# CristianSimion5/vk-raytracing-engine

Hardware: AMD Instinct MI355X
Metric: Mrays/s (higher is better)
Workload: dtype f32

## Files before the change

include/vkrt.h:

```cpp
#ifndef VKRT_H
#define VKRT_H

#include <stdint.h>
#include "vkrt_host_device.h"

#ifdef __cplusplus
extern "C" {
#endif

#define VKRT_ABI_VERSION 4

enum vkrt_status {
  VKRT_OK = 0,
  VKRT_ERR_INVALID_ARGUMENT = 1,
  VKRT_ERR_NO_DEVICE = 2,
  VKRT_ERR_HIP = 3,
  VKRT_ERR_OUT_OF_MEMORY = 4,
  VKRT_ERR_NOT_BUILT = 5,
  VKRT_ERR_UNSUPPORTED = 6
};

typedef struct vkrt_scene vkrt_scene;

typedef struct vkrt_prim_mesh {
// ... 88 lines not shown
  float    build_ms;
  uint64_t node_bytes;
  uint64_t triangle_bytes;
  uint32_t reference_count;
  uint32_t reserved;
} vkrt_accel_info;

int         vkrt_abi_version(void);
const char* vkrt_last_error(void);
int         vkrt_device_count(void);

int  vkrt_scene_create(const vkrt_scene_desc* desc, int device, vkrt_scene** out);
void vkrt_scene_destroy(vkrt_scene* scene);

enum vkrt_option {
  VKRT_OPT_MODE            = 1,
  VKRT_OPT_BVH_LAYOUT      = 2,
  VKRT_OPT_WF_SUBFRAMES    = 3,
  VKRT_OPT_WF_TRAV_BLOCK   = 4,
  VKRT_OPT_WF_SHARE        = 5,
  VKRT_OPT_TRI_THRESHOLD   = 6,
  VKRT_OPT_WF_SHARE_PERIOD = 7,
  VKRT_OPT_WF_SHARE_FLAGS  = 8,
  VKRT_OPT_GBUFFER_MIPS    = 9,
  VKRT_OPT_WATERTIGHT      = 10,
  VKRT_OPT_SKIP_DEAD_SHADOW_RAYS = 11,
  VKRT_OPT_ANYHIT_DISSOLVE = 12,
  VKRT_OPT_WF_FRAMES_IN_FLIGHT = 13,
  VKRT_OPT_SPLIT_BUDGET    = 14,
  VKRT_OPT_LAST            = 14,
  VKRT_OPT_WF_SAMPLE_SYNC  = 15,
  VKRT_OPT_WF_CAMERA_ROUNDS = 16,
  VKRT_OPT_WF_TRI_LEND = 17,
  VKRT_INFO_ANYHIT_ORDER   = 100,
  VKRT_INFO_SPLIT_BUDGET   = 101
};
int vkrt_scene_set_option(vkrt_scene* scene, int option, int value);
int vkrt_scene_get_option(const vkrt_scene* scene, int option, int* value);

int vkrt_accel_build(vkrt_scene* scene, uint32_t build_flags, void* hip_stream);
int vkrt_accel_get_info(const vkrt_scene* scene, vkrt_accel_info* out);

int vkrt_scene_update_nodes(vkrt_scene* scene, uint32_t first, uint32_t count, const vkrt_node* nodes, void* hip_stream);
int vkrt_accel_refit(vkrt_scene* scene, void* hip_stream);

enum vkrt_memory { VKRT_MEMORY_HOST = 0, VKRT_MEMORY_DEVICE = 1 };
typedef struct vkrt_vertex_update {
  uint32_t struct_size;
  uint32_t first, count;
  uint32_t memory;
  const float* positions;
  const float* normals;
  const float* tangents;
  const float* texcoords0;
} vkrt_vertex_update;
int vkrt_scene_update_vertices(vkrt_scene* scene, const vkrt_vertex_update* update, void* hip_stream);

typedef struct vkrt_ray {
  float origin[3];    float tmin;
  float direction[3]; float tmax;
} vkrt_ray;
typedef struct vkrt_hit {
  float   t, u, v;
  int32_t instance;
  int32_t primitive;
  int32_t prim_mesh;
// ... 154 lines not shown
```

vk-raytracing-engine_amd/abi.py:

```python
import ctypes as C

c_f = C.c_float
c_i = C.c_int32
c_u = C.c_uint32
c_u64 = C.c_uint64


class Mat4(C.Structure):
    _fields_ = [("m", c_f * 16)]


class GlobalUniforms(C.Structure):
    _fields_ = [("viewProj", Mat4), ("viewInverse", Mat4), ("projInverse", Mat4)]


class PushConstantRay(C.Structure):
    _fields_ = [
        ("clearColor", c_f * 4),
        ("frame", c_i),
        ("lightsCount", c_i),
        ("samples", c_i),
        ("depth", c_i),
        ("useShadows", c_i),
        ("useAO", c_i),
# ... 177 lines not shown
assert C.sizeof(VertexUpdate) == 48
assert C.sizeof(Ray) == 32
assert C.sizeof(Hit) == 32
assert C.sizeof(Surface) == 128
assert C.sizeof(InstanceVisibility) == 4
assert C.sizeof(QueryOpts) == 16
assert C.sizeof(MaterialAlpha) == 8

assert C.sizeof(GlobalUniforms) == 192
assert C.sizeof(PushConstantRay) == 44
assert C.sizeof(PrimMeshInfo) == 12
assert C.sizeof(GltfPBRMaterial) == 52
assert C.sizeof(GltfLight) == 32
assert C.sizeof(PrimMesh) == 20
assert C.sizeof(Node) == 68

VKRT_OK, VKRT_ERR_INVALID_ARGUMENT, VKRT_ERR_NO_DEVICE, VKRT_ERR_HIP, VKRT_ERR_OUT_OF_MEMORY, VKRT_ERR_NOT_BUILT, VKRT_ERR_UNSUPPORTED = range(7)
VKRT_BUILD_LBVH_GPU = 0x1
VKRT_BUILD_SAH_HOST = 0x2
VKRT_BUILD_PLOC_GPU = 0x4
VKRT_TRACE_SEED_INDEX_ROW_MAJOR = 0x1
VKRT_TRACE_COUNT_TRAVERSAL = 0x2
VKRT_TRACE_TIME_KERNELS = 0x4
VKRT_TRACE_SAME_SEED_EVERY_FRAME = 0x8
VKRT_ABI_VERSION = 4
VKRT_OPT_MODE, VKRT_OPT_BVH_LAYOUT, VKRT_OPT_WF_SUBFRAMES, VKRT_OPT_WF_TRAV_BLOCK = 1, 2, 3, 4
VKRT_OPT_WF_SHARE, VKRT_OPT_TRI_THRESHOLD, VKRT_OPT_WF_SHARE_PERIOD, VKRT_OPT_WF_SHARE_FLAGS = 5, 6, 7, 8
VKRT_OPT_GBUFFER_MIPS = 9
VKRT_OPT_WATERTIGHT, VKRT_OPT_SKIP_DEAD_SHADOW_RAYS, VKRT_OPT_ANYHIT_DISSOLVE = 10, 11, 12
VKRT_OPT_WF_FRAMES_IN_FLIGHT, VKRT_OPT_SPLIT_BUDGET = 13, 14
VKRT_OPT_WF_SAMPLE_SYNC = 15
VKRT_OPT_WF_CAMERA_ROUNDS = 16
VKRT_OPT_WF_TRI_LEND = 17
VKRT_INFO_ANYHIT_ORDER = 100
VKRT_INFO_SPLIT_BUDGET = 101
VKRT_INSTANCE_FACING_CULL_DISABLE, VKRT_INSTANCE_FLIP_FACING = 0x1, 0x2
VKRT_RAY_OPAQUE, VKRT_RAY_CULL_BACK_FACING, VKRT_RAY_CULL_FRONT_FACING = 0x1, 0x10, 0x20
VKRT_MEMORY_HOST, VKRT_MEMORY_DEVICE = 0, 1
VKRT_SURFACE_GEOMETRY, VKRT_SURFACE_MATERIAL = 0x1, 0x2
VKRT_ALPHA_OPAQUE, VKRT_ALPHA_MASK = 0, 1
VKRT_MULTIHIT_MAX = 16

VKRT_SYMBOLS = [
    "vkrt_abi_version",
    "vkrt_last_error",
    "vkrt_device_count",
    "vkrt_scene_create",
    "vkrt_scene_destroy",
    "vkrt_scene_set_option",
    "vkrt_scene_get_option",
    "vkrt_reserve",
    "vkrt_reserve_frames",
    "vkrt_accel_build",
    "vkrt_accel_get_info",
    "vkrt_scene_update_nodes",
    "vkrt_accel_refit",
    "vkrt_scene_update_vertices",
    "vkrt_intersect",
    "vkrt_occluded",
    "vkrt_scene_set_instance_visibility",
    "vkrt_scene_get_instance_visibility",
    "vkrt_intersect_ex",
    "vkrt_occluded_ex",
    "vkrt_intersect_multi",
    "vkrt_closest_point",
    "vkrt_hit_surface",
    "vkrt_scene_set_material_alpha",
    "vkrt_scene_get_material_alpha",
# ... 127 lines not shown
```

vk-raytracing-engine_amd/csrc/device_scene.h:

```cpp
#pragma once
#include <hip/hip_runtime.h>
#include <stddef.h>
#include <stdint.h>
#include "../../include/vkrt_host_device.h"
#include "device_math.h"

struct DevInstance
{
  float o2w[12];
  float w2o[9];
  int32_t primMesh;
  uint32_t vis;
  int32_t pad;
};
static_assert(sizeof(DevInstance) == 96, "DevInstance");
#define VKRT_VIS_CULL_DISABLE 0x100u
#define VKRT_VIS_FLIP 0x200u
#define VKRT_VIS_MIRRORED 0x10000u

#define VKRT_VERTEX_QUADS 3
#define VKRT_VERTEX_BYTES 48u
struct DevTexRef
{
  uint32_t offset;
// ... 88 lines not shown
#endif
#ifndef VKRT_W8_POSTPONE_ROOM
#define VKRT_W8_POSTPONE_ROOM 0
#endif

#define VKRT_COUNTER_SLOTS 64
struct DevCounters
{
  unsigned long long v[VKRT_COUNTER_SLOTS][VKRT_COUNTER_STRIDE];
};

#define VKRT_TRACE_PUBLIC_FLAGS 0xFu
#define VKRT_FLAG_SKIP_DEAD_SHADOW 0x100u
#define VKRT_FLAG_STORE_STAGED 0x200u
#define VKRT_FLAG_SAMPLE_SYNC 0x400u
#define VKRT_FLAG_CAMERA_ROUNDS 0x800u

struct TraceParams
{
  DevScene sc;
  PushConstantRay pc;
  float viewInverse[16];
  float projInverse[16];
  uint32_t seed;
  uint32_t flags;
  uint32_t fullW, fullH;
  uint32_t stripRows, shardCount, shardIndex;
  uint32_t localRows;
  uint32_t tilesX, tileCount;
  uint32_t tileFirst;
  float* image;
  unsigned int* workCounter;
  DevCounters* counters;
};

struct WfBuffers
{
  unsigned* ctrl;
  float4* planes;
  float4* stage;
  uint32_t capacity;
  uint32_t groups;
  float4* sampleState;
};
```

vk-raytracing-engine_amd/csrc/vkrt_api.cpp:

```cpp
#include <hip/hip_runtime.h>

#include <algorithm>
#include <chrono>
#include <cmath>
#include <cstdarg>
#include <cstdio>
#include <cstdlib>
#include <cstring>
#include <initializer_list>
#include <string>
#include <vector>

#include "../../include/vkrt.h"
#include "bvh_host.h"
#include "dev_buffer.h"
#include "device_scene.h"
#include "kernels.h"
#include "wide_node.h"

#define VKRT_TRI_THRESHOLD_DEFAULT 32
#define VKRT_WF_SHARE_DEFAULT 16
#define VKRT_WF_SHARE_FLAGS_DEFAULT 25
#define VKRT_WF_FRAMES_IN_FLIGHT_DEFAULT 3
#define VKRT_SPLIT_BUDGET_DEFAULT -1
#define VKRT_WF_SAMPLE_SYNC_DEFAULT 1
#define VKRT_WF_CAMERA_ROUNDS_DEFAULT 1
#define VKRT_WF_TRI_LEND_DEFAULT 1
#include "lbvh.h"
#include "refit.h"
#include "vertex_update.h"

namespace {

thread_local std::string g_lastError;

int fail(int code, const char* fmt, ...)
{
  char buf[512];
  va_list ap;
  va_start(ap, fmt);
  vsnprintf(buf, sizeof buf, fmt, ap);
  va_end(ap);
  g_lastError = buf;
  return code;
}

#define HIP_TRY(expr)                                                      \
  do                                                                       \
  {                                                                        \
    std::string m_;                                                        \
    if(const int rc_ = vkrt::hip_status((expr), #expr, m_); rc_ != VKRT_OK) \
      return fail(rc_, "%s", m_.c_str());                                  \
  } while(0)

}

struct vkrt_scene
{
  int device = 0;
  int cuCount = 256;
  std::vector<float> positions;
  std::vector<uint32_t> indices;
  std::vector<vkrt_prim_mesh> primMeshes;
  std::vector<vkrt_node> nodes;
  uint32_t lightCount = 0, materialCount = 0;
  std::vector<float> materialAlpha;
  std::vector<void*> allocs;
  DevScene dev{};
  vkrt::TreeBuffers accel;
  bool built = false;
  vkrt_accel_info info{};
  unsigned int* workCounter = nullptr;
  DevCounters* counters = nullptr;
  hipEvent_t evStart = nullptr, evStop = nullptr;
  bool timed = false;
  void* wfMem = nullptr;
  WfBuffers wf{};
  WfAsync wfAsync{};
  std::vector<hipEvent_t> wfEvents;
  WfTiming wfTiming{};
  bool wfTimed = false;
  int splitResolved = 0;
  int wfTimingRounds = 0;
  std::vector<hipEvent_t> wfPool;
  int opt[VKRT_OPT_WF_TRI_LEND + 1] = {0, 1, 1, 3, 64, VKRT_WF_SHARE_DEFAULT, VKRT_TRI_THRESHOLD_DEFAULT, 0, VKRT_WF_SHARE_FLAGS_DEFAULT, 1, 0, 0, 0,
                                            VKRT_WF_FRAMES_IN_FLIGHT_DEFAULT, VKRT_SPLIT_BUDGET_DEFAULT, VKRT_WF_SAMPLE_SYNC_DEFAULT, VKRT_WF_CAMERA_ROUNDS_DEFAULT,
                                      VKRT_WF_TRI_LEND_DEFAULT};
  bool hasLargeTriangles = false;
  bool wavefront = true;
  bool stale = false;
  bool refitted = false;
  vkrt::RefitScratch refit;
  bool positionsOnDevice = false;
  vkrt::DevBuf vertexStage;
  size_t vertexStageBytes = 0;
  std::vector<vkrt_instance_visibility> vis;
  uint64_t masksPresent[4] = {0, 0, 0, 0};
  vkrt::DevBuf nodeMasks;
  std::vector<vkrt_material_alpha> alpha;
  uint32_t alphaMasks = 0;
  const uint4* surfacePrimMeshes = nullptr;
};

namespace {

template <typename T>
int upload(vkrt_scene* s, const T* src, size_t count, const T** dst)
{
  void* p = nullptr;
  const size_t bytes = std::max<size_t>(count * sizeof(T), 16);
  HIP_TRY(hipMalloc(&p, bytes));
  s->allocs.push_back(p);
  if(count)
    HIP_TRY(hipMemcpy(p, src, count * sizeof(T), hipMemcpyHostToDevice));
  *dst = (const T*)p;
  return VKRT_OK;
}

int checkTransform(const vkrt_node& n, uint32_t i)
{
  for(int k = 0; k < 16; k++)
    if(!std::isfinite(n.worldMatrix[k]))
      return fail(VKRT_ERR_INVALID_ARGUMENT, "node %u: worldMatrix[%d] is not finite", i, k);
  return VKRT_OK;
}

int validate(const vkrt_scene_desc* d)
{
  if(!d)
    return fail(VKRT_ERR_INVALID_ARGUMENT, "desc is NULL");
  if(d->struct_size != sizeof(vkrt_scene_desc))
// ... 58 lines not shown
      const int x0 = cl((int)flx, (int)sw), x1 = cl((int)flx + 1, (int)sw), y0 = cl((int)fly, (int)sh), y1 = cl((int)fly + 1, (int)sh);
      const uint32_t p[4] = {src[(size_t)y0 * sw + x0], src[(size_t)y0 * sw + x1], src[(size_t)y1 * sw + x0], src[(size_t)y1 * sw + x1]};
      uint32_t out = 0;
      for(int c = 0; c < 4; c++)
      {
        const uint32_t base = (srgb && c < 3) ? 0u : 256u;
        const float t00 = lut512[base + ((p[0] >> (8 * c)) & 255u)], t10 = lut512[base + ((p[1] >> (8 * c)) & 255u)];
        const float t01 = lut512[base + ((p[2] >> (8 * c)) & 255u)], t11 = lut512[base + ((p[3] >> (8 * c)) & 255u)];
        float v = (t00 * (1.0f - ax) + t10 * ax) * (1.0f - ay) + (t01 * (1.0f - ax) + t11 * ax) * ay;
        if(srgb && c < 3) v = srgbEncode(v);
        v = v < 0.0f ? 0.0f : (v > 1.0f ? 1.0f : v);
        out |= (uint32_t)(v * 255.0f + 0.5f) << (8 * c);
      }
      dst[(size_t)y * dw + x] = out;
    }
}

bool useWavefront(const vkrt_scene* s) { return s->opt[VKRT_OPT_MODE] == 1; }

int clampOption(int option, int v)
{
  switch(option)
  {
    case VKRT_OPT_MODE: case VKRT_OPT_BVH_LAYOUT: return v ? 1 : 0;
    case VKRT_OPT_WF_SUBFRAMES: case VKRT_OPT_WF_FRAMES_IN_FLIGHT: return std::max(1, std::min(VKRT_WF_MAX_LANES, v));
    case VKRT_OPT_SPLIT_BUDGET: return std::max(-1, std::min(100, v));
    case VKRT_OPT_WF_TRAV_BLOCK: return v == 256 ? 256 : v == 128 ? 128 : 64;
    case VKRT_OPT_WF_SHARE: return std::max(0, std::min(64, v));
    case VKRT_OPT_TRI_THRESHOLD: return std::max(0, std::min(65, v));
    case VKRT_OPT_WF_SHARE_PERIOD: return std::max(0, std::min(255, v));
    case VKRT_OPT_WF_SHARE_FLAGS: return v & 31;
    case VKRT_OPT_GBUFFER_MIPS: case VKRT_OPT_WATERTIGHT: case VKRT_OPT_SKIP_DEAD_SHADOW_RAYS: case VKRT_OPT_ANYHIT_DISSOLVE: case VKRT_OPT_WF_SAMPLE_SYNC:
    case VKRT_OPT_WF_CAMERA_ROUNDS: case VKRT_OPT_WF_TRI_LEND: return v ? 1 : 0;
  }
  return v;
}

void optionsFromEnvironment(vkrt_scene* s)
{
  const char* e;
  if((e = getenv("VKRT_MODE")) && !strcmp(e, "mega")) s->opt[VKRT_OPT_MODE] = 0;
  if((e = getenv("VKRT_BVH")) && !strcmp(e, "bvh2")) s->opt[VKRT_OPT_BVH_LAYOUT] = 0;
  const struct { const char* name; int option; } ints[] = {{"VKRT_WF_SUBFRAMES", VKRT_OPT_WF_SUBFRAMES}, {"VKRT_WF_TRAV_BLOCK", VKRT_OPT_WF_TRAV_BLOCK},
                                                          {"VKRT_WF_SHARE", VKRT_OPT_WF_SHARE}, {"VKRT_TRI_THRESHOLD", VKRT_OPT_TRI_THRESHOLD},
                                                          {"VKRT_WF_SHARE_PERIOD", VKRT_OPT_WF_SHARE_PERIOD}, {"VKRT_WF_SHARE_FLAGS", VKRT_OPT_WF_SHARE_FLAGS},
                                                          {"VKRT_GBUFFER_MIPS", VKRT_OPT_GBUFFER_MIPS}, {"VKRT_WATERTIGHT", VKRT_OPT_WATERTIGHT},
                                                          {"VKRT_SKIP_DEAD_SHADOW_RAYS", VKRT_OPT_SKIP_DEAD_SHADOW_RAYS},
                                                          {"VKRT_ANYHIT_DISSOLVE", VKRT_OPT_ANYHIT_DISSOLVE}, {"VKRT_WF_FRAMES_IN_FLIGHT", VKRT_OPT_WF_FRAMES_IN_FLIGHT},
                                                          {"VKRT_SPLIT_BUDGET", VKRT_OPT_SPLIT_BUDGET}, {"VKRT_WF_SAMPLE_SYNC", VKRT_OPT_WF_SAMPLE_SYNC},
                                                          {"VKRT_WF_CAMERA_ROUNDS", VKRT_OPT_WF_CAMERA_ROUNDS},
                                                          {"VKRT_WF_TRI_LEND", VKRT_OPT_WF_TRI_LEND}};
  for(const auto& k : ints)
    if((e = getenv(k.name)))
      s->opt[k.option] = clampOption(k.option, atoi(e));
}

void freeAccel(vkrt_scene* s)
{
  s->accel = vkrt::TreeBuffers{};
  s->nodeMasks = vkrt::DevBuf{};
  s->built = false;
  s->refit = vkrt::RefitScratch{};
  s->refitted = false;
  s->stale = false;
}

constexpr vkrt_material_alpha kDefaultAlpha = {VKRT_ALPHA_OPAQUE, 0.5f};
constexpr vkrt_instance_visibility kDefaultVisibility = {0xFF, VKRT_INSTANCE_FACING_CULL_DISABLE, 0};

void makeInstance(const vkrt_node& node, const vkrt_instance_visibility& vis, DevInstance& in)
{
  memset(&in, 0, sizeof in);
  for(int r = 0; r < 3; r++)
    for(int c = 0; c < 4; c++)
      in.o2w[r * 4 + c] = node.worldMatrix[c * 4 + r];
  vkrt::invert3x3_rows(in.o2w, in.w2o);
  in.primMesh = node.primMesh;
  const float* m = in.o2w;
  const double det = (double)m[0] * ((double)m[5] * m[10] - (double)m[6] * m[9]) - (double)m[1] * ((double)m[4] * m[10] - (double)m[6] * m[8]) +
                     (double)m[2] * ((double)m[4] * m[9] - (double)m[5] * m[8]);
  in.vis = (uint32_t)vis.mask | ((uint32_t)vis.flags << 8) | (det < 0.0 ? VKRT_VIS_MIRRORED : 0u);
}

void noteMasks(vkrt_scene* s)
{
  memset(s->masksPresent, 0, sizeof s->masksPresent);
  for(const vkrt_instance_visibility& v : s->vis)
// ... 475 lines not shown
  *out = s;
  return VKRT_OK;
}

void vkrt_scene_destroy(vkrt_scene* s)
{
  if(!s)
    return;
  (void)hipSetDevice(s->device);
  freeAccel(s);
  for(void* p : s->allocs)
    (void)hipFree(p);
  if(s->wfMem) (void)hipFree(s->wfMem);
  if(s->wfAsync.count)
  {
    (void)hipEventDestroy(s->wfAsync.fork);
    for(int j = 0; j < s->wfAsync.count; j++)
    {
      (void)hipStreamDestroy(s->wfAsync.streams[j]);
      (void)hipEventDestroy(s->wfAsync.join[j]);
    }
  }
  for(hipEvent_t e : s->wfEvents) (void)hipEventDestroy(e);
  for(hipEvent_t e : s->wfPool) (void)hipEventDestroy(e);
  if(s->evStart) (void)hipEventDestroy(s->evStart);
  if(s->evStop) (void)hipEventDestroy(s->evStop);
  delete s;
}

int vkrt_scene_set_option(vkrt_scene* s, int option, int value)
{
  if(!s)
    return fail(VKRT_ERR_INVALID_ARGUMENT, "scene is NULL");
  if(option < VKRT_OPT_MODE || option > VKRT_OPT_WF_TRI_LEND)
    return fail(VKRT_ERR_INVALID_ARGUMENT, "unknown option %d", option);
  if(clampOption(option, value) != value)
    return fail(VKRT_ERR_INVALID_ARGUMENT, "option %d: value %d out of range", option, value);
  s->opt[option] = value;
  if(option == VKRT_OPT_WF_TRI_LEND && s->built && s->dev.layout == 1u)
    s->dev.shareFlags = (s->dev.shareFlags & ~VKRT_SHARE_TRI_LEND) | (value ? VKRT_SHARE_TRI_LEND : 0u);
  return VKRT_OK;
}

int vkrt_scene_get_option(const vkrt_scene* s, int option, int* value)
{
  if(!s || !value)
    return fail(VKRT_ERR_INVALID_ARGUMENT, "NULL argument");
  if(option == VKRT_INFO_ANYHIT_ORDER)
  {
    *value = s->built ? (int)(s->dev.shareFlags & 6u) : 0;
    return VKRT_OK;
  }
  if(option == VKRT_INFO_SPLIT_BUDGET)
  {
    *value = s->built ? s->splitResolved : 0;
    return VKRT_OK;
  }
  if(option < VKRT_OPT_MODE || option > VKRT_OPT_WF_TRI_LEND)
    return fail(VKRT_ERR_INVALID_ARGUMENT, "unknown option %d", option);
  *value = s->opt[option];
  return VKRT_OK;
}

int vkrt_reserve(vkrt_scene* s, const vkrt_shard* shard, void* hip_stream)
{
  if(!s)
    return fail(VKRT_ERR_INVALID_ARGUMENT, "NULL argument");
  return vkrt_reserve_frames(s, shard, (uint32_t)std::max(1, s->opt[VKRT_OPT_WF_FRAMES_IN_FLIGHT]), hip_stream);
}

int vkrt_reserve_frames(vkrt_scene* s, const vkrt_shard* shard, uint32_t frames_per_call, void* hip_stream)
{
  if(!s || !shard)
    return fail(VKRT_ERR_INVALID_ARGUMENT, "NULL argument");
  if(frames_per_call == 0)
    return fail(VKRT_ERR_INVALID_ARGUMENT, "frames_per_call is 0");
  int rc = checkShard(shard);
  if(rc == VKRT_OK)
    rc = setDevice(s);
  if(rc != VKRT_OK)
    return rc;
  const uint64_t tiles = (uint64_t)((shard->full_width + 7) / 8) * ((vkrt_shard_rows(shard) + 7) / 8);
  if(tiles * 64 >= 0xFFFFFFFFull)
    return fail(VKRT_ERR_UNSUPPORTED, "launch too large");
  const bool wavefront = s->built ? s->wavefront : useWavefront(s);
  if(tiles == 0 || !wavefront)
    return VKRT_OK;
  int rc2 = ensureWorkingSet(s, (uint32_t)tiles * 64u, framesInFlight(s, (int)std::min<uint32_t>(frames_per_call, VKRT_FRAMES_PER_BATCH)), (hipStream_t)hip_stream);
  if(rc2 == VKRT_OK)
    rc2 = ensureEventPool(s, (int)std::min<uint32_t>(frames_per_call, VKRT_FRAMES_PER_BATCH));
  return rc2;
// ... 203 lines not shown
      std::vector<float> records((size_t)r.triCount * 12);
      hipError_t e = hipSuccess;
      if(r.tree.nodeCount) e = hipMemcpy(b2.nodes.data(), r.tree.buf.nodes.get(), b2.nodes.size() * 4, hipMemcpyDeviceToHost);
      if(e == hipSuccess) e = hipMemcpy(records.data(), r.tree.buf.tris.get(), records.size() * 4, hipMemcpyDeviceToHost);
      r.tree.buf = vkrt::TreeBuffers{};
      if(e != hipSuccess)
        return fail(VKRT_ERR_HIP, "LBVH download: %s", hipGetErrorString(e));
      b2.rootRef = r.tree.rootRef;
      b2.maxDepth = r.tree.maxDepth;
      b2.triOrder.resize(r.triCount);
      std::vector<vkrt::FlatTri> tris(r.triCount);
      for(uint32_t k = 0; k < r.triCount; k++)
      {
        b2.triOrder[k] = k;
        tris[k] = vkrt::unpack_triangle(&records[(size_t)k * 12], watertight);
      }
      vkrt::BuiltWide8 w8;
      vkrt::collapse_wide8(b2, tris, w8, watertight);
      if((rc = uploadHostTree(s, tris, nullptr, &w8, dissolvePtr, stream, tree)) != VKRT_OK)
        return rc;
    }
    else
      tree = std::move(r.tree);
  }
  installTree(s, tree);
  sceneBounds(s);
  if((rc = traversalSettings(s)) != VKRT_OK)
    return rc;
  if(s->dev.layout == 1u)
  {
    HIP_TRY(s->nodeMasks.alloc(std::max<size_t>(s->info.node_bytes / VKRT_WNODE_BYTES * 8, 16)));
    if((rc = computeNodeMasks(s, stream)) != VKRT_OK)
      return rc;
  }
  s->info.build_ms = std::chrono::duration<float, std::milli>(std::chrono::steady_clock::now() - t0).count();
  s->built = true;
  return VKRT_OK;
}

}

int vkrt_accel_build(vkrt_scene* s, uint32_t flags, void* hip_stream)
{
  if(!s)
    return fail(VKRT_ERR_INVALID_ARGUMENT, "scene is NULL");
  hipStream_t stream = (hipStream_t)hip_stream;
  if(s->positionsOnDevice)
  {
    int rc = setDevice(s);
    if(rc != VKRT_OK)
      return rc;
    HIP_TRY(hipDeviceSynchronize());
    if(!s->positions.empty())
      HIP_TRY(hipMemcpy(s->positions.data(), s->dev.positions, s->positions.size() * sizeof(float), hipMemcpyDeviceToHost));
    s->positionsOnDevice = false;
  }
  const bool deviceBuild = flags == 0 || (flags & (VKRT_BUILD_LBVH_GPU | VKRT_BUILD_PLOC_GPU)) != 0;
  if(s->opt[VKRT_OPT_SPLIT_BUDGET] >= 0 || !deviceBuild)
  {
    s->splitResolved = std::max(0, s->opt[VKRT_OPT_SPLIT_BUDGET]);
    return accelBuildOnce(s, flags, s->splitResolved, stream);
  }
  const auto t0 = std::chrono::steady_clock::now();
  float sahSplit = 0.0f;
  int rc = accelBuildOnce(s, flags, 30, stream);
  if(rc == VKRT_OK)
// ... 330 lines not shown
  int rc = checkBuilt(s, "vkrt_pathtrace");
  if(rc == VKRT_OK)
    rc = checkShard(shard);
  if(rc != VKRT_OK)
    return rc;
  if(pc->lightsCount < 0 || (uint32_t)pc->lightsCount > s->lightCount)
    return fail(VKRT_ERR_INVALID_ARGUMENT, "PushConstantRay.lightsCount %d outside [0,%u]", pc->lightsCount, s->lightCount);
  if(pc->samples < 0 || pc->depth < 0 || pc->depth > 99)
    return fail(VKRT_ERR_INVALID_ARGUMENT, "samples/depth out of range");
  if((rc = setDevice(s)) != VKRT_OK)
    return rc;
  hipStream_t stream = (hipStream_t)hip_stream;
  TraceParams P;
  if((rc = launchParams(s, pc, cam, opts, shard, P)) != VKRT_OK)
    return rc;
  if(P.localRows == 0)
    return VKRT_OK;
  if(s->opt[VKRT_OPT_SKIP_DEAD_SHADOW_RAYS])
    P.flags |= VKRT_FLAG_SKIP_DEAD_SHADOW;
  P.image = image;
  P.workCounter = s->workCounter;

  const bool count = (P.flags & VKRT_TRACE_COUNT_TRAVERSAL) != 0;
  if(s->wavefront)
  {
    if(P.fullW > 65535u || P.localRows > 65535u || pc->samples > 65535)
      return fail(VKRT_ERR_UNSUPPORTED, "wavefront mode packs pixel coordinates / sample index in 16 bits");
    const uint32_t seedStep = (P.flags & VKRT_TRACE_SAME_SEED_EVERY_FRAME) ? 0u : 1u;
    if(s->opt[VKRT_OPT_WF_SAMPLE_SYNC])
      P.flags |= VKRT_FLAG_SAMPLE_SYNC;
    if(s->opt[VKRT_OPT_WF_CAMERA_ROUNDS] && (P.flags & VKRT_FLAG_SAMPLE_SYNC) && s->dev.layout == 1u && travBlock(s) == 64 && s->dev.shareMinIdle != 0u &&
       s->dev.triThreshold != 0u)
      P.flags |= VKRT_FLAG_CAMERA_ROUNDS;
    if((rc = ensureWorkingSet(s, P.tileCount * 64u, framesInFlight(s, (int)n_frames), stream)) != VKRT_OK)
      return rc;
    if((rc = ensureEventPool(s, (int)std::min<uint32_t>(n_frames, VKRT_FRAMES_PER_BATCH))) != VKRT_OK)
      return rc;
    WfTiming* timing = nullptr;
    if(P.flags & VKRT_TRACE_TIME_KERNELS)
    {
      const size_t wantEv = (size_t)2 * (2 * (size_t)pc->samples * pc->depth) * std::min<uint32_t>(n_frames, 8u);
      while(s->wfEvents.size() < wantEv && s->wfEvents.size() < 8192)
      {
        hipEvent_t e;
        HIP_TRY(hipEventCreate(&e));
        s->wfEvents.push_back(e);
      }
      s->wfTiming.events = s->wfEvents.data();
      s->wfTiming.capacity = (int)s->wfEvents.size();
      timing = &s->wfTiming;
    }
    s->wfTimed = timing != nullptr;
    s->wfTimingRounds = (pc->samples > 0 && pc->depth > 0) ? pc->samples * (pc->depth + 1) : 0;
    HIP_TRY(hipEventRecord(s->evStart, stream));
    WfOptions wo;
    wo.subframes = s->opt[VKRT_OPT_WF_SUBFRAMES];
    wo.travBlock = travBlock(s);
    wo.inFlight = framesInFlight(s, (int)n_frames);
    if(timing)
      timing->used = 0;
    for(uint32_t first = 0; first < n_frames; first += VKRT_FRAMES_PER_BATCH)
    {
      TraceParams Pb = P;
      Pb.pc.frame = P.pc.frame + (int)first;
      Pb.seed = P.seed + first * seedStep;
      HIP_TRY(vkrt_launch_wavefront(Pb, s->wf, wo, (int)std::min<uint32_t>(VKRT_FRAMES_PER_BATCH, n_frames - first), seedStep, count, stream, timing, &s->wfAsync));
// ... 678 lines not shown
```

vk-raytracing-engine_amd/csrc/wf_traverse.hip:

```cpp
#include <hip/hip_runtime.h>

#include "device_math.h"
#include "device_scene.h"
#include "kernels.h"
#include "rgen.h"
#include "traverse.h"
#include "traverse_wide.h"
#include "traverse_share.h"
#include "wf_streams.h"

enum { WF_K_CLOSEST_C = 0, WF_K_CLOSEST_P = 1, WF_K_SHADOW_S = 2, WF_K_SHADOW_P = 3 };

VKRT_DEV void storeHit(const TraceParams& P, const WfBuffers& B, int par, int kind, unsigned qi, const RayHit& hit)
{
  if(kind == WF_K_SHADOW_S)
    wfStore(rec(B, par, WF_S, WF_H0, qi), make_float4(0.0f, 0.0f, 0.0f, __int_as_float(hit.slot >= 0 ? 0 : -1)));
  else if(kind == WF_K_SHADOW_P)
    ((float*)rec(B, par, WF_P, WF_H0, qi))[0] = __int_as_float(hit.slot >= 0 ? 1 : 0);
  else
  {
    const int type = kind == WF_K_CLOSEST_C ? WF_C : WF_P;
    int inst = -1;
    if(hit.slot >= 0)
    {
      const uint4 ts = P.sc.triShade[hit.slot];
      inst = __float_as_int(P.sc.tris[hit.slot * VKRT_TRI_QUADS + 2].z);
      wfStore(rec(B, par, type, WF_H1, qi), make_float4(__uint_as_float(ts.x), __uint_as_float(ts.y), __uint_as_float(ts.z), __uint_as_float(ts.w)));
    }
    float* h = (float*)rec(B, par, type, WF_H0, qi);
    if(type == WF_C)
      wfStore(rec(B, par, WF_C, WF_H0, qi), make_float4(hit.t, hit.u, hit.v, __int_as_float(inst)));
    else
    {
      h[1] = hit.u; h[2] = hit.v; h[3] = __int_as_float(inst);
    }
  }
}

template <bool COUNT, bool WIDE, int TB, int TM = 0>
__global__ __launch_bounds__(TB)
__attribute__((amdgpu_waves_per_eu(TM != 0 && WIDE && TB == 64 ? 5 : 1)))
void k_wf_traverse(const TraceParams P, const WfBuffers B, const int round)
{
  extern __shared__ int lds_stack[];
  const int par = round & 1;
  const unsigned cC = *countOf(B, par, WF_C), cS = *countOf(B, par, WF_S), cP = *countOf(B, par, WF_P);
  if(blockIdx.x == 0 && threadIdx.x == 0)
  {
    for(int t = 0; t < WF_TYPES; t++) *countOf(B, par ^ 1, t) = 0u;
    if(cC + cP) atomicAdd(&P.counters->v[round % VKRT_COUNTER_SLOTS][0], (unsigned long long)cC + cP);
    if(cS + cP) atomicAdd(&P.counters->v[round % VKRT_COUNTER_SLOTS][1], (unsigned long long)cS + cP);
    if(cP) atomicAdd(&P.counters->v[round % VKRT_COUNTER_SLOTS][11], (unsigned long long)cP);
  }
  const unsigned nC = (cC + TB - 1) / TB, nP = (cP + TB - 1) / TB, nS = (cS + TB - 1) / TB;
  unsigned blk = blockIdx.x;
  int kind;
  unsigned count;
  if(blk < nC) { kind = WF_K_CLOSEST_C; count = cC; }
  else if((blk -= nC) < nP) { kind = WF_K_CLOSEST_P; count = cP; }
  else if((blk -= nP) < nS) { kind = WF_K_SHADOW_S; count = cS; }
  else if((blk -= nS) < nP) { kind = WF_K_SHADOW_P; count = cP; }
  else return;
  const bool anyHit = kind >= WF_K_SHADOW_S;
  const int type = kind == WF_K_CLOSEST_C ? WF_C : kind == WF_K_SHADOW_S ? WF_S : WF_P;
  const unsigned qi = blk * TB + threadIdx.x;
  const bool valid = qi < count;
  float4 r0 = make_float4(0.0f, 0.0f, 0.0f, 0.0f), r1 = make_float4(1.0f, 0.0f, 0.0f, 0.0f);
  if(valid)
  {
    r0 = wfLoad(rec(B, par, type, WF_R0, qi));
    r1 = wfLoad(rec(B, par, type, kind == WF_K_CLOSEST_P ? WF_R2 : WF_R1, qi));
    if(kind == WF_K_CLOSEST_P)
      r0.w = 10000.0f;
  }
  uint32_t raySeed = 0u;
  if((TM & VKRT_TM_DISSOLVE) && valid)
    raySeed = __float_as_uint(wfLoad(rec(B, par, type, WF_S0, qi)).w);
  TravCount tc;
  __shared__ int shareLds[VKRT_SHARE_LDS_WORDS];
  RayHit hit;
  if(WIDE && TB == 64 && P.sc.shareMinIdle != 0u && P.sc.triThreshold != 0u)
  {
    uint2* stk = ((uint2*)lds_stack) + threadIdx.x;
    if(anyHit)
      traverse_wide8_share<COUNT, true, TM>(P.sc, valid, mk3(r0.x, r0.y, r0.z), mk3(r1.x, r1.y, r1.z), 0.001f, r0.w, stk, shareRes(shareLds), hit, tc, raySeed);
    else
      traverse_wide8_share<COUNT, false, TM>(P.sc, valid, mk3(r0.x, r0.y, r0.z), mk3(r1.x, r1.y, r1.z), 0.001f, r0.w, stk, shareRes(shareLds), hit, tc, raySeed);
    if(valid)
      storeHit(P, B, par, kind, qi, hit);
  }
  else if(valid)
  {
    traverse_any<COUNT, WIDE, TM>(P.sc, mk3(r0.x, r0.y, r0.z), mk3(r1.x, r1.y, r1.z), 0.001f, r0.w, anyHit, lds_stack, (int)threadIdx.x, TB, hit, tc, raySeed);
    storeHit(P, B, par, kind, qi, hit);
  }
  if(COUNT)
  {
    __shared__ unsigned long long red[VKRT_COUNTER_STRIDE * (TB / 64)];
    const unsigned vals[10] = {0, 0, 0, 0, 0, 0, tc.nodes, tc.tris, tc.waveNodeSteps, tc.waveTriSteps};
    blockAddCounters(&P.counters->v[blockIdx.x % VKRT_COUNTER_SLOTS][0], vals, 10, red);
  }
}

template <bool COUNT, int TM>
__global__ __launch_bounds__(64)
__attribute__((amdgpu_waves_per_eu(TM != 0 ? 5 : 1)))
void k_wf_traverse_camera(const TraceParams P, const WfBuffers B, const int round, const int smpl)
{
  extern __shared__ int lds_stack[];
  const int par = round & 1;
  if(blockIdx.x == 0 && threadIdx.x == 0)
    for(int t = 0; t < WF_TYPES; t++) *countOf(B, par ^ 1, t) = 0u;
  const unsigned w = blockIdx.x * 64u + threadIdx.x;
  uint32_t x = 0, y = 0, lrow = 0;
  const bool valid = pixelOfWork(P, w, P.tileFirst, x, y, lrow);
  f3 o = mk3(0.0f), d = mk3(1.0f, 0.0f, 0.0f);
  uint32_t raySeed = 0u;
  if(valid)
  {
    LaneState L;
    bindPixel(P, L, x, lrow);
    L.prd.seed = smpl == 0 ? pixelSeed(P, x, y) : __float_as_uint(((const float*)(B.sampleState + pixelSlot(P, x, lrow)))[3]);
// ... 61 lines not shown
```

vk-raytracing-engine_amd/renderer.py:

```python
import ctypes as C
import os

import numpy as np

from . import LIB_PATH, abi

_lib = None


def load_library():
    global _lib
    if _lib is None:
        import torch

        if not os.path.exists(LIB_PATH):
            raise RuntimeError(f"{LIB_PATH} missing: build it with __graft_entry__.build() "
                               "(there is no CPU fallback for the ray-tracing path)")
        _lib = abi.declare_vkrt(C.CDLL(LIB_PATH))
        if _lib.vkrt_abi_version() != abi.VKRT_ABI_VERSION:
            raise RuntimeError("libvkrt.so ABI version mismatch")
    return _lib


ALPHA_OPAQUE, ALPHA_MASK = abi.VKRT_ALPHA_OPAQUE, abi.VKRT_ALPHA_MASK
# ... 339 lines not shown
            accum = torch.zeros((rows, width, 4), dtype=torch.float32, device=f"cuda:{self.device}")
        stream = stream or torch.cuda.current_stream(accum.device)
        gb = abi.Gbuffer(*(gbuffer[k].data_ptr() for k in ("color", "position", "normal", "roughMetal")))
        opts = abi.TraceOpts(seed & 0xFFFFFFFF, flags)
        if "nrdViewZ" in gbuffer:
            nrd = abi.NrdPlanes(gbuffer["nrdNormalRoughness"].data_ptr(), gbuffer["nrdViewZ"].data_ptr(), gbuffer["nrdRadianceHitDist"].data_ptr())
            _check(self.lib.vkrt_hybrid_trace_nrd(self._h, C.byref(pc), C.byref(cam), C.byref(opts), C.byref(shard), C.byref(gb), C.byref(nrd),
                                                  C.c_void_p(accum.data_ptr()), C.c_void_p(stream.cuda_stream)), "vkrt_hybrid_trace_nrd")
            return accum
        _check(self.lib.vkrt_hybrid_trace(self._h, C.byref(pc), C.byref(cam), C.byref(opts), C.byref(shard), C.byref(gb),
                                          C.c_void_p(accum.data_ptr()), C.c_void_p(stream.cuda_stream)), "vkrt_hybrid_trace")
        return accum

    def post(self, main_img, rt_img=None, rt_mode=0, view_accumulated=0, use_gi=0, stream=None):
        import torch

        out = torch.empty_like(main_img)
        stream = stream or torch.cuda.current_stream(main_img.device)
        pcp = abi.PushConstantPost(1.0, rt_mode, view_accumulated, use_gi)
        _check(self.lib.vkrt_post(self.device, C.byref(pcp), main_img.numel() // 4, C.c_void_p(main_img.data_ptr()),
                                  C.c_void_p(rt_img.data_ptr()) if rt_img is not None else None, C.c_void_p(out.data_ptr()),
                                  C.c_void_p(stream.cuda_stream)), "vkrt_post")
        return out

    def reset_counters(self, stream=None):
        _check(self.lib.vkrt_counters_reset(self._h, C.c_void_p(stream.cuda_stream) if stream is not None else None),
               "vkrt_counters_reset")

    def counters(self):
        c = abi.Counters()
        _check(self.lib.vkrt_counters_read(self._h, C.byref(c)), "vkrt_counters_read")
        return c.as_dict()

    def last_trace_ms(self):
        ms = C.c_float()
        _check(self.lib.vkrt_last_trace_ms(self._h, C.byref(ms)), "vkrt_last_trace_ms")
        return float(ms.value)

    def last_trace_timing(self):
        t = abi.TraceTiming()
        _check(self.lib.vkrt_last_trace_timing(self._h, C.byref(t)), "vkrt_last_trace_timing")
        return {"total_ms": float(t.total_ms), "traverse_ms": float(t.traverse_ms), "traverse_launches": int(t.traverse_launches),
                "mode": "wavefront" if t.mode == 1 else "megakernel", "shade_ms": float(t.shade_ms), "shade_launches": int(t.shade_launches)}

    def _query_args(self, rays, what):
        import torch

        if not isinstance(rays, torch.Tensor):
            raise VkrtError(f"{what}: rays must be a torch tensor (pack_rays), got {type(rays).__name__}")
        if not rays.is_cuda:
            raise VkrtError(f"{what}: rays are on {rays.device}, the scene is on cuda:{self.device}")
        if rays.device.index != self.device:
            raise VkrtError(f"{what}: rays are on {rays.device}, the scene is on cuda:{self.device}")
        if rays.dtype != torch.float32:
            raise VkrtError(f"{what}: rays are {rays.dtype}, expected torch.float32")
        if rays.dim() != 2 or rays.shape[1] != 8:
            raise VkrtError(f"{what}: rays have shape {tuple(rays.shape)}, expected [N, 8]")
        if not rays.is_contiguous() or rays.data_ptr() % 16 != 0:
            raise VkrtError(f"{what}: rays must be contiguous and 16-byte aligned")
        if rays.shape[0] >= 1 << 32:
            raise VkrtError(f"{what}: {rays.shape[0]} rays, at most 2^32 - 1 per call")
        return int(rays.shape[0])

    def _query_out(self, out, shape, what, align):
        import torch

# ... 243 lines not shown
```

Baseline: 5433.

## Add per-light direction-hashed shadow occluder cache to skip any-hit traversal

Adds a device hash table keyed by the nearest light and an octahedral-quantised ray direction, which records the last triangle that occluded a shadow ray. Before traversal, an any-hit ray tests the cached triangle with a full ray-triangle test, including the culling and any-hit checks. If that triangle occludes the ray, the ray skips BVH traversal entirely; otherwise it traverses and writes its occluder back to the table. This aims to cut shadow-ray traversal cost, at the price of an extra hashed global load per ray and atomic stores that race across rays. The stored hit carries tmax and zero barycentrics rather than the real hit attributes.

```diff
diff --git a/include/vkrt.h b/include/vkrt.h
--- a/include/vkrt.h
+++ b/include/vkrt.h
@@ -144,6 +144,8 @@
   VKRT_OPT_WF_SAMPLE_SYNC  = 15,
   VKRT_OPT_WF_CAMERA_ROUNDS = 16,
   VKRT_OPT_WF_TRI_LEND = 17,
+  VKRT_OPT_WF_SHADOW_CACHE = 18,
+  VKRT_INFO_SHADOW_CACHE_RESOLVED = 102,
   VKRT_INFO_ANYHIT_ORDER   = 100,
   VKRT_INFO_SPLIT_BUDGET   = 101
 };
diff --git a/vk-raytracing-engine_amd/abi.py b/vk-raytracing-engine_amd/abi.py
--- a/vk-raytracing-engine_amd/abi.py
+++ b/vk-raytracing-engine_amd/abi.py
@@ -233,8 +233,10 @@
 VKRT_OPT_WF_SAMPLE_SYNC = 15
 VKRT_OPT_WF_CAMERA_ROUNDS = 16
 VKRT_OPT_WF_TRI_LEND = 17
+VKRT_OPT_WF_SHADOW_CACHE = 18
 VKRT_INFO_ANYHIT_ORDER = 100
 VKRT_INFO_SPLIT_BUDGET = 101
+VKRT_INFO_SHADOW_CACHE_RESOLVED = 102
 VKRT_INSTANCE_FACING_CULL_DISABLE, VKRT_INSTANCE_FLIP_FACING = 0x1, 0x2
 VKRT_RAY_OPAQUE, VKRT_RAY_CULL_BACK_FACING, VKRT_RAY_CULL_FRONT_FACING = 0x1, 0x10, 0x20
 VKRT_MEMORY_HOST, VKRT_MEMORY_DEVICE = 0, 1
diff --git a/vk-raytracing-engine_amd/csrc/device_scene.h b/vk-raytracing-engine_amd/csrc/device_scene.h
--- a/vk-raytracing-engine_amd/csrc/device_scene.h
+++ b/vk-raytracing-engine_amd/csrc/device_scene.h
@@ -144,7 +144,12 @@
   float* image;
   unsigned int* workCounter;
   DevCounters* counters;
+  uint32_t* shadowCache;
+  uint32_t shadowCacheMask;
+  uint32_t shadowCacheRes;
 };
+#define VKRT_SHADOW_CACHE_MAX_LIGHTS 16
+#define VKRT_COUNTER_SHADOW_CACHE 12
 
 struct WfBuffers
 {
diff --git a/vk-raytracing-engine_amd/csrc/vkrt_api.cpp b/vk-raytracing-engine_amd/csrc/vkrt_api.cpp
--- a/vk-raytracing-engine_amd/csrc/vkrt_api.cpp
+++ b/vk-raytracing-engine_amd/csrc/vkrt_api.cpp
@@ -26,6 +26,9 @@
 #define VKRT_WF_SAMPLE_SYNC_DEFAULT 1
 #define VKRT_WF_CAMERA_ROUNDS_DEFAULT 1
 #define VKRT_WF_TRI_LEND_DEFAULT 1
+#define VKRT_WF_SHADOW_CACHE_DEFAULT 1
+#define VKRT_SHADOW_CACHE_BITS_DEFAULT 22
+#define VKRT_SHADOW_CACHE_RES_DEFAULT 1024
 #include "lbvh.h"
 #include "refit.h"
 #include "vertex_update.h"
@@ -83,9 +86,9 @@
   int splitResolved = 0;
   int wfTimingRounds = 0;
   std::vector<hipEvent_t> wfPool;
-  int opt[VKRT_OPT_WF_TRI_LEND + 1] = {0, 1, 1, 3, 64, VKRT_WF_SHARE_DEFAULT, VKRT_TRI_THRESHOLD_DEFAULT, 0, VKRT_WF_SHARE_FLAGS_DEFAULT, 1, 0, 0, 0,
+  int opt[VKRT_OPT_WF_SHADOW_CACHE + 1] = {0, 1, 1, 3, 64, VKRT_WF_SHARE_DEFAULT, VKRT_TRI_THRESHOLD_DEFAULT, 0, VKRT_WF_SHARE_FLAGS_DEFAULT, 1, 0, 0, 0,
                                             VKRT_WF_FRAMES_IN_FLIGHT_DEFAULT, VKRT_SPLIT_BUDGET_DEFAULT, VKRT_WF_SAMPLE_SYNC_DEFAULT, VKRT_WF_CAMERA_ROUNDS_DEFAULT,
-                                      VKRT_WF_TRI_LEND_DEFAULT};
+                                      VKRT_WF_TRI_LEND_DEFAULT, VKRT_WF_SHADOW_CACHE_DEFAULT};
   bool hasLargeTriangles = false;
   bool wavefront = true;
   bool stale = false;
@@ -97,6 +100,9 @@
   std::vector<vkrt_instance_visibility> vis;
   uint64_t masksPresent[4] = {0, 0, 0, 0};
   vkrt::DevBuf nodeMasks;
+  vkrt::DevBuf shadowCache;
+  uint32_t shadowCacheBits = VKRT_SHADOW_CACHE_BITS_DEFAULT, shadowCacheRes = VKRT_SHADOW_CACHE_RES_DEFAULT;
+  uint32_t shadowCacheEntries = 0;
   std::vector<vkrt_material_alpha> alpha;
   uint32_t alphaMasks = 0;
   const uint4* surfacePrimMeshes = nullptr;
@@ -221,6 +227,7 @@
     case VKRT_OPT_WF_SHARE_FLAGS: return v & 31;
     case VKRT_OPT_GBUFFER_MIPS: case VKRT_OPT_WATERTIGHT: case VKRT_OPT_SKIP_DEAD_SHADOW_RAYS: case VKRT_OPT_ANYHIT_DISSOLVE: case VKRT_OPT_WF_SAMPLE_SYNC:
     case VKRT_OPT_WF_CAMERA_ROUNDS: case VKRT_OPT_WF_TRI_LEND: return v ? 1 : 0;
+    case VKRT_OPT_WF_SHADOW_CACHE: return std::max(0, std::min(2, v));
   }
   return v;
 }
@@ -238,10 +245,20 @@
                                                           {"VKRT_ANYHIT_DISSOLVE", VKRT_OPT_ANYHIT_DISSOLVE}, {"VKRT_WF_FRAMES_IN_FLIGHT", VKRT_OPT_WF_FRAMES_IN_FLIGHT},
                                                           {"VKRT_SPLIT_BUDGET", VKRT_OPT_SPLIT_BUDGET}, {"VKRT_WF_SAMPLE_SYNC", VKRT_OPT_WF_SAMPLE_SYNC},
                                                           {"VKRT_WF_CAMERA_ROUNDS", VKRT_OPT_WF_CAMERA_ROUNDS},
-                                                          {"VKRT_WF_TRI_LEND", VKRT_OPT_WF_TRI_LEND}};
+                                                          {"VKRT_WF_TRI_LEND", VKRT_OPT_WF_TRI_LEND},
+                                                          {"VKRT_WF_SHADOW_CACHE", VKRT_OPT_WF_SHADOW_CACHE}};
   for(const auto& k : ints)
     if((e = getenv(k.name)))
       s->opt[k.option] = clampOption(k.option, atoi(e));
+  if((e = getenv("VKRT_WF_SHADOW_CACHE_BITS")))
+    s->shadowCacheBits = (uint32_t)std::max(10, std::min(26, atoi(e)));
+  if((e = getenv("VKRT_WF_SHADOW_CACHE_RES")))
+  {
+    uint32_t r = 16u;
+    while(r < 4096u && r < (uint32_t)std::max(0, atoi(e)))
+      r *= 2u;
+    s->shadowCacheRes = r;
+  }
 }
 
 void freeAccel(vkrt_scene* s)
@@ -783,7 +800,7 @@
 {
   if(!s)
     return fail(VKRT_ERR_INVALID_ARGUMENT, "scene is NULL");
-  if(option < VKRT_OPT_MODE || option > VKRT_OPT_WF_TRI_LEND)
+  if(option < VKRT_OPT_MODE || option > VKRT_OPT_WF_SHADOW_CACHE)
     return fail(VKRT_ERR_INVALID_ARGUMENT, "unknown option %d", option);
   if(clampOption(option, value) != value)
     return fail(VKRT_ERR_INVALID_ARGUMENT, "option %d: value %d out of range", option, value);
@@ -807,7 +824,19 @@
     *value = s->built ? s->splitResolved : 0;
     return VKRT_OK;
   }
-  if(option < VKRT_OPT_MODE || option > VKRT_OPT_WF_TRI_LEND)
+  if(option == VKRT_INFO_SHADOW_CACHE_RESOLVED)
+  {
+    HIP_TRY(hipSetDevice(s->device));
+    HIP_TRY(hipDeviceSynchronize());
+    std::vector<unsigned long long> h(sizeof(DevCounters) / sizeof(unsigned long long));
+    HIP_TRY(hipMemcpy(h.data(), s->counters, sizeof(DevCounters), hipMemcpyDeviceToHost));
+    unsigned long long n = 0;
+    for(int sl = 0; sl < VKRT_COUNTER_SLOTS; sl++)
+      n += h[(size_t)sl * VKRT_COUNTER_STRIDE + VKRT_COUNTER_SHADOW_CACHE];
+    *value = (int)std::min<unsigned long long>(n, 0x7fffffffull);
+    return VKRT_OK;
+  }
+  if(option < VKRT_OPT_MODE || option > VKRT_OPT_WF_SHADOW_CACHE)
     return fail(VKRT_ERR_INVALID_ARGUMENT, "unknown option %d", option);
   *value = s->opt[option];
   return VKRT_OK;
@@ -1077,6 +1106,15 @@
     HIP_TRY(s->nodeMasks.alloc(std::max<size_t>(s->info.node_bytes / VKRT_WNODE_BYTES * 8, 16)));
     if((rc = computeNodeMasks(s, stream)) != VKRT_OK)
       return rc;
+    if(s->wavefront)
+    {
+      if(s->shadowCacheEntries == 0u)
+      {
+        HIP_TRY(s->shadowCache.alloc(sizeof(uint32_t) << s->shadowCacheBits));
+        s->shadowCacheEntries = 1u << s->shadowCacheBits;
+      }
+      HIP_TRY(hipMemsetAsync(s->shadowCache.get(), 0xFF, sizeof(uint32_t) * (size_t)s->shadowCacheEntries, stream));
+    }
   }
   s->info.build_ms = std::chrono::duration<float, std::milli>(std::chrono::steady_clock::now() - t0).count();
   s->built = true;
@@ -1473,6 +1511,13 @@
     if(s->opt[VKRT_OPT_WF_CAMERA_ROUNDS] && (P.flags & VKRT_FLAG_SAMPLE_SYNC) && s->dev.layout == 1u && travBlock(s) == 64 && s->dev.shareMinIdle != 0u &&
        s->dev.triThreshold != 0u)
       P.flags |= VKRT_FLAG_CAMERA_ROUNDS;
+    if(s->opt[VKRT_OPT_WF_SHADOW_CACHE] >= (count ? 2 : 1) && s->shadowCacheEntries != 0u && s->dev.layout == 1u && travBlock(s) == 64 &&
+       s->dev.shareMinIdle != 0u && s->dev.triThreshold != 0u && pc->lightsCount <= VKRT_SHADOW_CACHE_MAX_LIGHTS)
+    {
+      P.shadowCache = s->shadowCache.get<uint32_t>();
+      P.shadowCacheMask = s->shadowCacheEntries - 1u;
+      P.shadowCacheRes = s->shadowCacheRes;
+    }
     if((rc = ensureWorkingSet(s, P.tileCount * 64u, framesInFlight(s, (int)n_frames), stream)) != VKRT_OK)
       return rc;
     if((rc = ensureEventPool(s, (int)std::min<uint32_t>(n_frames, VKRT_FRAMES_PER_BATCH))) != VKRT_OK)
diff --git a/vk-raytracing-engine_amd/csrc/wf_traverse.hip b/vk-raytracing-engine_amd/csrc/wf_traverse.hip
--- a/vk-raytracing-engine_amd/csrc/wf_traverse.hip
+++ b/vk-raytracing-engine_amd/csrc/wf_traverse.hip
@@ -35,6 +35,39 @@
       h[1] = hit.u; h[2] = hit.v; h[3] = __int_as_float(inst);
     }
   }
+}
+
+VKRT_DEV unsigned shadowCacheIndex(const TraceParams& P, f3 o, f3 d, float tmax)
+{
+  const float te = tmax + 0.1f;
+  const f3 e = mk3(fmaf(d.x, te, o.x), fmaf(d.y, te, o.y), fmaf(d.z, te, o.z));
+  unsigned light = 0u;
+  float best = 3.0e38f;
+  for(int k = 0; k < P.pc.lightsCount; k++)
+  {
+    const float lx = P.sc.lights[k].position[0] - e.x, ly = P.sc.lights[k].position[1] - e.y, lz = P.sc.lights[k].position[2] - e.z;
+    const float d2 = (lx * lx + ly * ly) + lz * lz;
+    if(d2 < best)
+    {
+      best = d2;
+      light = (unsigned)k;
+    }
+  }
+  const float inv = 1.0f / fmaxf((fabsf(d.x) + fabsf(d.y)) + fabsf(d.z), 1e-30f);
+  float px = -d.x * inv, py = -d.y * inv;
+  if(d.z > 0.0f)
+  {
+    const float qx = copysignf(1.0f - fabsf(py), px), qy = copysignf(1.0f - fabsf(px), py);
+    px = qx; py = qy;
+  }
+  const float R = (float)P.shadowCacheRes;
+  const unsigned cx = (unsigned)fminf(fmaxf((px * 0.5f + 0.5f) * R, 0.0f), R - 1.0f);
+  const unsigned cy = (unsigned)fminf(fmaxf((py * 0.5f + 0.5f) * R, 0.0f), R - 1.0f);
+  unsigned h = ((light << 20) | ((cy >> 2) << 10) | (cx >> 2)) * 0x9E3779B1u;
+  h ^= h >> 15;
+  h *= 0x85EBCA77u;
+  h ^= h >> 13;
+  return ((h << 4) | ((cy & 3u) << 2) | (cx & 3u)) & P.shadowCacheMask;
 }
 
 template <bool COUNT, bool WIDE, int TB, int TM = 0>
@@ -83,11 +116,58 @@
   {
     uint2* stk = ((uint2*)lds_stack) + threadIdx.x;
     if(anyHit)
-      traverse_wide8_share<COUNT, true, TM>(P.sc, valid, mk3(r0.x, r0.y, r0.z), mk3(r1.x, r1.y, r1.z), 0.001f, r0.w, stk, shareRes(shareLds), hit, tc, raySeed);
+    {
+      constexpr bool CACHE = (TM & (VKRT_TM_WATERTIGHT | VKRT_TM_DISSOLVE)) != (VKRT_TM_WATERTIGHT | VKRT_TM_DISSOLVE);
+      const bool cacheOn = CACHE && P.shadowCache != nullptr;
+      bool walks = valid;
+      unsigned ci = 0u;
+      if(cacheOn)
+      {
+        bool resolved = false;
+        if(valid)
+        {
+          const f3 o = mk3(r0.x, r0.y, r0.z), d = mk3(r1.x, r1.y, r1.z);
+          ci = shadowCacheIndex(P, o, d, r0.w);
+          const unsigned s = __hip_atomic_load(&P.shadowCache[ci], __ATOMIC_RELAXED, __HIP_MEMORY_SCOPE_AGENT);
+          if(s < P.sc.triCount)
+          {
+            const float4* __restrict__ tp = P.sc.tris + (size_t)s * VKRT_TRI_QUADS;
+            const float4 a = tp[0];
+            const float4 b = tp[1];
+            const float4 c = tp[2];
+            TriRay<(TM & VKRT_TM_WATERTIGHT) != 0> tr;
+            tr.set(d);
+            float t, u, v;
+            bool ccw;
+            resolved = tr.hit(o, d, a, b, c, t, u, v, ccw) && t > 0.001f && t < r0.w && !query_rejects<TM>(P.sc, c, ccw) &&
+                       !anyhit_ignores<TM>(P.sc, s, c.y, raySeed, VKRT_HOOK_UV(TM, u, v));
+            if(resolved)
+            {
+              RayHit pre;
+              pre.t = r0.w; pre.u = 0.0f; pre.v = 0.0f; pre.slot = (int)s;
+              storeHit(P, B, par, kind, qi, pre);
+            }
+          }
+        }
+        const unsigned nResolved = (unsigned)__popcll(__ballot(resolved));
+        if(threadIdx.x == 0 && nResolved)
+          atomicAdd(&P.counters->v[blockIdx.x % VKRT_COUNTER_SLOTS][VKRT_COUNTER_SHADOW_CACHE], (unsigned long long)nResolved);
+        walks = valid && !resolved;
+      }
+      traverse_wide8_share<COUNT, true, TM>(P.sc, walks, mk3(r0.x, r0.y, r0.z), mk3(r1.x, r1.y, r1.z), 0.001f, r0.w, stk, shareRes(shareLds), hit, tc, raySeed);
+      if(walks)
+      {
+        storeHit(P, B, par, kind, qi, hit);
+        if(cacheOn && hit.slot >= 0)
+          __hip_atomic_store(&P.shadowCache[ci], (unsigned)hit.slot, __ATOMIC_RELAXED, __HIP_MEMORY_SCOPE_AGENT);
+      }
+    }
     else
+    {
       traverse_wide8_share<COUNT, false, TM>(P.sc, valid, mk3(r0.x, r0.y, r0.z), mk3(r1.x, r1.y, r1.z), 0.001f, r0.w, stk, shareRes(shareLds), hit, tc, raySeed);
-    if(valid)
-      storeHit(P, B, par, kind, qi, hit);
+      if(valid)
+        storeHit(P, B, par, kind, qi, hit);
+    }
   }
   else if(valid)
   {
diff --git a/vk-raytracing-engine_amd/renderer.py b/vk-raytracing-engine_amd/renderer.py
--- a/vk-raytracing-engine_amd/renderer.py
+++ b/vk-raytracing-engine_amd/renderer.py
@@ -395,6 +395,9 @@
         _check(self.lib.vkrt_counters_read(self._h, C.byref(c)), "vkrt_counters_read")
         return c.as_dict()
 
+    def shadow_cache_resolved(self):
+        return self.get_option(abi.VKRT_INFO_SHADOW_CACHE_RESOLVED)
+
     def last_trace_ms(self):
         ms = C.c_float()
         _check(self.lib.vkrt_last_trace_ms(self._h, C.byref(ms)), "vkrt_last_trace_ms")
```

Result: no change. 5468, median of 6 (+0.6%).
